# manoskary/analysisgnn

Measured on AMD Instinct MI355X. Metric: subgraph-nodes/sec fwd+bwd, HybridGNN L=3 H=256, higher is better.
Workload: dtype f32; 1 GPU; C2 (sampled, the batch a training step sees): HybridGNN L=3 H=256 out=128, 21 task heads, 32 neighbour-sampled subgraphs x (500 target notes + [5,5] hops) per GPU, per-hop counts passed (every layer trimmed); 16335 notes, 104099 edges per GPU; train step = fwd + objective (wloss) + bwd + allreduce + clip + AdamW, CSR rebuilt every step; hipGraph replay; workload_id=c2s, per_gpu_subgraphs=32, objective=wloss, parallelism=dp1, allreduce=none (one rank)

## Files before the change

### analysisgnn_amd/csrc/wgrad.hip

```cpp
#include "agnn_common.h"

namespace {

using agnn::f32x16;

struct WgArgs {
  const float* dy;
  const float* x;
  int64_t ld_dy, ld_x;
  int32_t n, out_f, in_f;
  int32_t rows_per_slice;
  int32_t tiles_in;
  float* slab;
  float* slab_b;
  int32_t out_pad, in_pad;
};

__device__ __forceinline__ void wgrad_tile(const WgArgs& a, const int tile, const int slice) {
  const int lane = threadIdx.x & 63;
  const int wave = threadIdx.x >> 6;
  const int wm = wave >> 1, wn = wave & 1;
  const int to = tile / a.tiles_in, ti = tile - to * a.tiles_in;
  const int kk = lane >> 5, c32 = lane & 31;
  const int ocol = to * 128 + wm * 64 + 2 * c32;
  const int icol = ti * 128 + wn * 64 + 2 * c32;
  const bool o_ok = ocol < a.out_f;
  const bool i_ok = icol < a.in_f;
  const int r0 = slice * a.rows_per_slice;
  int r1 = r0 + a.rows_per_slice;
  if (r1 > a.n) r1 = a.n;

  f32x16 acc00 = {0}, acc01 = {0}, acc10 = {0}, acc11 = {0};
  float bs0 = 0.f, bs1 = 0.f;
  const float* dy_s = a.dy + static_cast<int64_t>(r0) * a.ld_dy;
  const float* x_s = a.x + static_cast<int64_t>(r0) * a.ld_x;
  const uint32_t ldb_dy = static_cast<uint32_t>(a.ld_dy) * 4u, ldb_x = static_cast<uint32_t>(a.ld_x) * 4u;
  const uint32_t cb_dy = (o_ok ? ocol : 0) * 4u, cb_x = (i_ok ? icol : 0) * 4u;
  const int rel_last = a.n - 1 - r0;
  constexpr int CH = 8;
  constexpr int STEP = 2 * CH;
  float2 a0[CH], b0[CH], a1[CH], b1[CH], a2[CH], b2[CH];
  uint32_t o_dy = static_cast<uint32_t>(kk) * ldb_dy + cb_dy, o_x = static_cast<uint32_t>(kk) * ldb_x + cb_x;
  const uint32_t s_dy = 2u * ldb_dy, s_x = 2u * ldb_x;
  auto fetch_fast = [&](float2* ao, float2* bo) {
#pragma unroll
    for (int u = 0; u < CH; ++u) {
      ao[u] = *reinterpret_cast<const float2*>(reinterpret_cast<const char*>(dy_s) + o_dy);
      bo[u] = *reinterpret_cast<const float2*>(reinterpret_cast<const char*>(x_s) + o_x);
      o_dy += s_dy;
      o_x += s_x;
    }
    __builtin_amdgcn_sched_barrier(0);
  };
// ... 46 lines not shown
    fetch_fast(a1, b1);
    mma(a2, b2);
  }
  for (; c + 3 <= nfull; c += 3) {
    fetch(c + 2, a2, b2);
    mma(a0, b0);
    fetch(c + 3, a0, b0);
    mma(a1, b1);
    fetch(c + 4, a1, b1);
    mma(a2, b2);
  }
  fetch(c + 2, a2, b2);
  if (c < nchunks) mma_tail(c, a0, b0);
  if (c + 1 < nchunks) mma_tail(c + 1, a1, b1);
  if (c + 2 < nchunks) mma_tail(c + 2, a2, b2);
  float* slab = a.slab + (static_cast<int64_t>(slice) * a.out_pad) * a.in_pad;
  const int ob = to * 128 + wm * 64, ib = ti * 128 + wn * 64;
#pragma unroll
  for (int r = 0; r < 16; ++r) {
    const int i = agnn::d_row32(r, kk);
    float* row0 = slab + static_cast<int64_t>(ob + 2 * i) * a.in_pad + ib + 2 * c32;
    float* row1 = row0 + a.in_pad;
    *reinterpret_cast<float2*>(row0) = make_float2(acc00[r], acc01[r]);
    *reinterpret_cast<float2*>(row1) = make_float2(acc10[r], acc11[r]);
  }
  if (a.slab_b != nullptr && wn == 0) {
    bs0 += __shfl_xor(bs0, 32, 64);
    bs1 += __shfl_xor(bs1, 32, 64);
    if (kk == 0 && ti == 0)
      *reinterpret_cast<float2*>(a.slab_b + static_cast<int64_t>(slice) * a.out_pad + ocol) = make_float2(bs0, bs1);
  }
}

__global__ __launch_bounds__(256) void k_wgrad(WgArgs a) { wgrad_tile(a, blockIdx.x, blockIdx.y); }

constexpr int kWgBatchMax = AGNN_WGRAD_BATCH_MAX_ITEMS;

struct WgBatch {
  WgArgs it[kWgBatchMax];
  int32_t first[kWgBatchMax + 1];
  int32_t tiles[kWgBatchMax];
  int32_t n;
};

__global__ __launch_bounds__(256) void k_wgrad_batch(WgBatch b) {
  int i = 0;
  const int blk = blockIdx.x;
  while (i + 1 < b.n && blk >= b.first[i + 1]) ++i;
  const int local = blk - b.first[i];
  const int tiles = b.tiles[i];
  const int slice = local / tiles;
  wgrad_tile(b.it[i], local - slice * tiles, slice);
}


template <typename StoreW, typename StoreB>
__device__ __forceinline__ void wgrad_reduce_sums(const float* __restrict__ slab, const float* __restrict__ slab_b, int S, int out_f, int in_f,
                                                  int out_pad, int in_pad, const bool with_bias, const int block, const int n_blocks,
                                                  StoreW store_w, StoreB store_b) {
  __shared__ float2 part[8][32];
  const int col = threadIdx.x & 31, sg = threadIdx.x >> 5;
  const int half_in = in_f >> 1;
  const int64_t total = static_cast<int64_t>(out_f) * half_in;
  const int64_t plane = static_cast<int64_t>(out_pad) * in_pad;
  for (int64_t e0 = static_cast<int64_t>(block) * 32; e0 < total; e0 += static_cast<int64_t>(n_blocks) * 32) {
    const int64_t e = e0 + col;
    float2 s = make_float2(0.f, 0.f);
    int o = 0, i = 0;
    if (e < total) {
      o = static_cast<int>(e / half_in);
      i = static_cast<int>(e - static_cast<int64_t>(o) * half_in) * 2;
      const float* p = slab + static_cast<int64_t>(o) * in_pad + i;
      for (int k = sg; k < S; k += 8) {
        const float2 v = *reinterpret_cast<const float2*>(p + k * plane);
        s.x += v.x;
        s.y += v.y;
      }
    }
    part[sg][col] = s;
    __syncthreads();
    if (sg == 0 && e < total) {
      float2 t = part[0][col];
#pragma unroll
      for (int g = 1; g < 8; ++g) { t.x += part[g][col].x; t.y += part[g][col].y; }
      store_w(o, i, t);
// ... 61 lines not shown
};

Plan make_plan(int64_t n, int out_f, int in_f) {
  Plan p;
  p.tiles_out = (out_f + 127) / 128;
  p.tiles_in = (in_f + 127) / 128;
  p.out_pad = p.tiles_out * 128;
  p.in_pad = p.tiles_in * 128;
  const int tiles = p.tiles_out * p.tiles_in;
  int64_t S = 512 / tiles;
  const int64_t max_s = (n + 63) / 64;
  if (S > max_s) S = max_s;
  if (S > 64) S = 64;
  if (S < 1) S = 1;
  int64_t rps = (n + S - 1) / S;
  rps = (rps + 1) & ~int64_t{1};
  p.rows_per_slice = static_cast<int>(rps);
  p.S = static_cast<int>((n + rps - 1) / rps);
  return p;
}

}

int agnn::launch_slab_reduce(const float* slab, const float* slab_b, int S, int out_f, int in_f, int out_pad, int in_pad,
                             float* dw, int64_t ld_dw, float* db, hipStream_t s) {
  const int64_t total = static_cast<int64_t>(out_f) * (in_f >> 1);
  int blocks = static_cast<int>((total + 31) / 32);
  if (blocks > 4096) blocks = 4096;
  if (blocks < 1) blocks = 1;
  hipLaunchKernelGGL(k_wgrad_reduce, dim3(blocks), dim3(256), 0, s, slab, slab_b, S, out_f, in_f, out_pad, in_pad, dw, ld_dw, db);
  return check_launch("slab_reduce");
}

extern "C" size_t agnn_wgrad_workspace_bytes(int64_t n, int32_t out_f, int32_t in_f) {
  if (n <= 0 || out_f <= 0 || in_f <= 0) return 0;
  const Plan p = make_plan(n, out_f, in_f);
  return (static_cast<size_t>(p.S) * p.out_pad * p.in_pad + static_cast<size_t>(p.S) * p.out_pad) * sizeof(float) + 256;
}

extern "C" int agnn_wgrad_f32(const float* dy, int64_t ld_dy, const float* x, int64_t ld_x, int64_t n, int32_t out_f,
                              int32_t in_f, float* dw, int64_t ld_dw, float* db, void* workspace, size_t workspace_bytes,
                              agnn_stream_t stream_) {
  using namespace agnn;
  if (n <= 0 || n >= (int64_t{1} << 31) || out_f <= 0 || in_f <= 0) return fail(AGNN_EINVAL, "wgrad: bad sizes n=%lld out=%d in=%d", (long long)n, out_f, in_f);
  if ((out_f & 1) || (in_f & 1) || (ld_dy & 1) || (ld_x & 1) || (ld_dw & 1)) return fail(AGNN_EALIGN, "wgrad: widths and leading dimensions must be even");
  if (!dy || !x || !dw || !workspace) return fail(AGNN_EINVAL, "wgrad: null argument");
  if ((reinterpret_cast<uintptr_t>(dy) | reinterpret_cast<uintptr_t>(x) | reinterpret_cast<uintptr_t>(dw) | reinterpret_cast<uintptr_t>(db)) & 7u)
    return fail(AGNN_EALIGN, "wgrad: pointers must be 8-byte aligned");
  if (ld_dy < out_f || ld_x < in_f || ld_dw < in_f) return fail(AGNN_EINVAL, "wgrad: leading dimension smaller than the width");
  const size_t need = agnn_wgrad_workspace_bytes(n, out_f, in_f);
  if (workspace_bytes < need) return fail(AGNN_ENOMEM, "wgrad: workspace %zu < %zu bytes", workspace_bytes, need);
  const Plan p = make_plan(n, out_f, in_f);
  if ((static_cast<int64_t>(p.rows_per_slice) + 128) * (ld_dy > ld_x ? ld_dy : ld_x) * 4 >= (int64_t{1} << 32))
    return fail(AGNN_EINVAL, "wgrad: a row slice (%d rows x ld) exceeds the kernel's 32-bit byte offsets", p.rows_per_slice);
  char* ws = reinterpret_cast<char*>((reinterpret_cast<uintptr_t>(workspace) + 255) & ~uintptr_t{255});
  float* slab = reinterpret_cast<float*>(ws);
  float* slab_b = slab + static_cast<size_t>(p.S) * p.out_pad * p.in_pad;
  WgArgs a{dy, x, ld_dy, ld_x, static_cast<int32_t>(n), out_f, in_f, p.rows_per_slice, p.tiles_in, slab,
           db ? slab_b : nullptr, p.out_pad, p.in_pad};
  hipStream_t s = static_cast<hipStream_t>(stream_);
  hipLaunchKernelGGL(k_wgrad, dim3(p.tiles_out * p.tiles_in, p.S), dim3(256), 0, s, a);
  if (int rc = check_launch("wgrad")) return rc;
  return launch_slab_reduce(slab, db ? slab_b : nullptr, p.S, out_f, in_f, p.out_pad, p.in_pad, dw, ld_dw, db, s);
}

namespace {
struct BatchPlan {
  int n;
  int tiles_out[kWgBatchMax], tiles_in[kWgBatchMax], S[kWgBatchMax], rps[kWgBatchMax];
  size_t slab_off[kWgBatchMax], slabb_off[kWgBatchMax], total_floats;
};

int batch_plan(int n_items, const agnn_wgrad_item_t* items, BatchPlan& bp) {
  using namespace agnn;
  if (n_items <= 0 || n_items > kWgBatchMax || !items) return fail(AGNN_EINVAL, "wgrad_batch: %d items (1 .. %d)", n_items, kWgBatchMax);
  bp.n = n_items;
  int64_t tiles = 0;
  for (int i = 0; i < n_items; ++i) {
    const agnn_wgrad_item_t& it = items[i];
    if (it.n <= 0 || it.n >= (int64_t{1} << 31) || it.out_f <= 0 || it.in_f <= 0) return fail(AGNN_EINVAL, "wgrad_batch: item %d: bad sizes", i);
    bp.tiles_out[i] = (it.out_f + 127) / 128;
    bp.tiles_in[i] = (it.in_f + 127) / 128;
    tiles += static_cast<int64_t>(bp.tiles_out[i]) * bp.tiles_in[i];
  }
  int64_t S = 384 / tiles;
  if (S > 64) S = 64;
  if (S < 1) S = 1;
  size_t off = 0;
  for (int i = 0; i < n_items; ++i) {
    const agnn_wgrad_item_t& it = items[i];
    int64_t s_i = S;
    const int64_t max_s = (it.n + 63) / 64;
    if (s_i > max_s) s_i = max_s;
    int64_t rps = (it.n + s_i - 1) / s_i;
// ... 25 lines not shown
  if (int rc = batch_plan(n_items, items, bp)) return rc;
  if (!workspace || workspace_bytes < bp.total_floats * sizeof(float) + 256) return fail(AGNN_ENOMEM, "wgrad_batch: workspace too small");
  float* ws = reinterpret_cast<float*>((reinterpret_cast<uintptr_t>(workspace) + 255) & ~uintptr_t{255});
  WgBatch wb{};
  RedBatch rb{};
  wb.n = rb.n = n_items;
  int wg = 0, red = 0;
  for (int i = 0; i < n_items; ++i) {
    const agnn_wgrad_item_t& it = items[i];
    if ((it.out_f & 1) || (it.in_f & 1) || (it.ld_dy & 1) || (it.ld_x & 1) || (it.ld_dw & 1)) return fail(AGNN_EALIGN, "wgrad_batch: item %d: widths and leading dimensions must be even", i);
    if (!it.dy || !it.x || !it.dw) return fail(AGNN_EINVAL, "wgrad_batch: item %d: null argument", i);
    if ((reinterpret_cast<uintptr_t>(it.dy) | reinterpret_cast<uintptr_t>(it.x) | reinterpret_cast<uintptr_t>(it.dw) | reinterpret_cast<uintptr_t>(it.db)) & 7u)
      return fail(AGNN_EALIGN, "wgrad_batch: item %d: pointers must be 8-byte aligned", i);
    if (it.ld_dy < it.out_f || it.ld_x < it.in_f || it.ld_dw < it.in_f) return fail(AGNN_EINVAL, "wgrad_batch: item %d: leading dimension smaller than the width", i);
    if ((static_cast<int64_t>(bp.rps[i]) + 128) * (it.ld_dy > it.ld_x ? it.ld_dy : it.ld_x) * 4 >= (int64_t{1} << 32))
      return fail(AGNN_EINVAL, "wgrad_batch: item %d: a row slice (%d rows x ld) exceeds the kernel's 32-bit byte offsets", i, bp.rps[i]);
    const int out_pad = bp.tiles_out[i] * 128, in_pad = bp.tiles_in[i] * 128;
    float* slab = ws + bp.slab_off[i];
    float* slab_b = ws + bp.slabb_off[i];
    wb.it[i] = WgArgs{it.dy, it.x, it.ld_dy, it.ld_x, static_cast<int32_t>(it.n), it.out_f, it.in_f, bp.rps[i], bp.tiles_in[i], slab,
                      it.db ? slab_b : nullptr, out_pad, in_pad};
    wb.tiles[i] = bp.tiles_out[i] * bp.tiles_in[i];
    wb.first[i] = wg;
    wg += wb.tiles[i] * bp.S[i];
    rb.it[i] = RedItem{slab, it.db ? slab_b : nullptr, it.dw, it.db, it.ld_dw, bp.S[i], it.out_f, it.in_f, out_pad, in_pad};
    rb.first[i] = red;
    int64_t blocks = (static_cast<int64_t>(it.out_f) * (it.in_f >> 1) + 31) / 32;
    if (blocks > 1024) blocks = 1024;
    red += static_cast<int>(blocks);
  }
  wb.first[n_items] = wg;
  rb.first[n_items] = red;
  hipStream_t s = static_cast<hipStream_t>(stream_);
  hipLaunchKernelGGL(k_wgrad_batch, dim3(static_cast<unsigned>(wg)), dim3(256), 0, s, wb);
  if (int rc = check_launch("wgrad_batch")) return rc;
  hipLaunchKernelGGL(k_wgrad_reduce_batch, dim3(static_cast<unsigned>(red)), dim3(256), 0, s, rb);
  return check_launch("wgrad_batch(reduce)");
}

namespace {

constexpr int kEpiRecMax = 64;
constexpr int kEpiDbMax = 48;
constexpr int kEpiSumMax = AGNN_GRAD_MAX_SUMS;
constexpr int kEpiPartRows = 1024;

struct EpiRec {
  float* p;
  int32_t ld, c0, c1, scalar;
};
struct EpiItem {
  const float* slab;
  const float* slab_b;
  int32_t S, out_f, in_f, out_pad, in_pad;
  int16_t rec0, rec1, db0, db1;
};
struct EpiSum {
  const float* part;
  float* dgamma;
  float* dbeta;
  int32_t n_rows, H;
};
struct EpiBatch {
  EpiItem it[kWgBatchMax];
  EpiRec rec[kEpiRecMax];
  float* db[kEpiDbMax];
  EpiSum sum[kEpiSumMax];
  int32_t first[kWgBatchMax + kEpiSumMax + 1];
// ... 70 lines not shown
  int64_t ld;
  int32_t rows, cols;
  int32_t item, c0, c1;
};

bool spans_overlap(const EpiSpan& a, const EpiSpan& b) {
  const float* a_end = a.p + static_cast<int64_t>(a.rows - 1) * a.ld + a.cols;
  const float* b_end = b.p + static_cast<int64_t>(b.rows - 1) * b.ld + b.cols;
  if (a_end <= b.p || b_end <= a.p) return false;
  if (a.rows > 1 && b.rows > 1 && a.ld == b.ld) {
    int64_t r = (b.p - a.p) % a.ld;
    if (r < 0) r += a.ld;
    if (r >= a.cols && r + b.cols <= a.ld) return false;
  }
  return true;
}

}

static void epi_as_wgrad(int32_t n_items, const agnn_grad_item_t* items, agnn_wgrad_item_t* out) {
  for (int i = 0; i < n_items; ++i) {
    const agnn_grad_item_t& g = items[i];
    out[i] = agnn_wgrad_item_t{g.dy, g.x, nullptr, nullptr, g.ld_dy, g.ld_x, g.in_f, g.n, g.out_f, g.in_f};
  }
}

extern "C" size_t agnn_grad_epilogue_workspace_bytes(int32_t n_items, const agnn_grad_item_t* items) {
  if (n_items <= 0 || n_items > kWgBatchMax || !items) return 0;
  agnn_wgrad_item_t w[kWgBatchMax];
  epi_as_wgrad(n_items, items, w);
  return agnn_wgrad_batch_workspace_bytes(n_items, w);
}

extern "C" int agnn_grad_epilogue_f32(int32_t n_items, const agnn_grad_item_t* items, int32_t n_sums, const agnn_colsum_item_t* sums,
                                      void* workspace, size_t workspace_bytes, agnn_stream_t stream_) {
  using namespace agnn;
  if (n_items < 0 || n_items > kWgBatchMax || (n_items > 0 && !items)) return fail(AGNN_EINVAL, "grad_epilogue: %d products (0 .. %d)", n_items, kWgBatchMax);
  if (n_sums < 0 || n_sums > kEpiSumMax || (n_sums > 0 && !sums)) return fail(AGNN_EINVAL, "grad_epilogue: %d column sums (0 .. %d)", n_sums, kEpiSumMax);
  if (n_items == 0 && n_sums == 0) return AGNN_OK;
  BatchPlan bp;
  bp.n = 0;
  bp.total_floats = 0;
  float* ws = nullptr;
  if (n_items > 0) {
    agnn_wgrad_item_t w[kWgBatchMax];
    epi_as_wgrad(n_items, items, w);
    if (int rc = batch_plan(n_items, w, bp)) return rc;
    if (!workspace || workspace_bytes < bp.total_floats * sizeof(float) + 256) return fail(AGNN_ENOMEM, "grad_epilogue: workspace too small");
    ws = reinterpret_cast<float*>((reinterpret_cast<uintptr_t>(workspace) + 255) & ~uintptr_t{255});
  }
  static thread_local EpiSpan spans[kWgBatchMax * 2 * AGNN_PACK_MAX_SRC + 2 * kEpiSumMax];
  int n_spans = 0;
  for (int i = 0; i < n_items; ++i) {
    const agnn_grad_item_t& it = items[i];
    if ((it.out_f & 1) || (it.in_f & 1) || (it.ld_dy & 1) || (it.ld_x & 1)) return fail(AGNN_EALIGN, "grad_epilogue: item %d: widths and leading dimensions must be even", i);
    if (!it.dy || !it.x) return fail(AGNN_EINVAL, "grad_epilogue: item %d: null argument", i);
    if ((reinterpret_cast<uintptr_t>(it.dy) | reinterpret_cast<uintptr_t>(it.x)) & 7u) return fail(AGNN_EALIGN, "grad_epilogue: item %d: pointers must be 8-byte aligned", i);
    if (it.ld_dy < it.out_f || it.ld_x < it.in_f) return fail(AGNN_EINVAL, "grad_epilogue: item %d: leading dimension smaller than the width", i);
    if ((static_cast<int64_t>(bp.rps[i]) + 128) * (it.ld_dy > it.ld_x ? it.ld_dy : it.ld_x) * 4 >= (int64_t{1} << 32))
      return fail(AGNN_EINVAL, "grad_epilogue: item %d: a row slice (%d rows x ld) exceeds the kernel's 32-bit byte offsets", i, bp.rps[i]);
    if (it.n_dw < 0 || it.n_dw > AGNN_PACK_MAX_SRC || it.n_db < 0 || it.n_db > AGNN_PACK_MAX_SRC || it.n_dw + it.n_db == 0)
      return fail(AGNN_EINVAL, "grad_epilogue: item %d: %d weight and %d bias destinations (0 .. %d each, one at least)", i, it.n_dw, it.n_db, AGNN_PACK_MAX_SRC);
    for (int k = 0; k < it.n_dw; ++k) {
      const agnn_grad_dst_t& d = it.dw[k];
      const int cols = d.c1 - d.c0;
      if (!d.p || d.c0 < 0 || cols <= 0 || d.c1 > it.in_f || d.ld < cols || d.ld >= (int64_t{1} << 31))
        return fail(AGNN_EINVAL, "grad_epilogue: item %d: destination %d: columns [%d, %d) of %d, ld %lld", i, k, d.c0, d.c1, it.in_f, (long long)d.ld);
      if (reinterpret_cast<uintptr_t>(d.p) & 3u) return fail(AGNN_EALIGN, "grad_epilogue: item %d: destination %d is not a float pointer", i, k);
      if (!(cols & 1) && ((d.c0 & 1) || (d.ld & 1) || (reinterpret_cast<uintptr_t>(d.p) & 7u)))
        return fail(AGNN_EALIGN, "grad_epilogue: item %d: destination %d: an even column block needs an even c0, an even ld and an 8-byte aligned pointer", i, k);
      spans[n_spans++] = EpiSpan{d.p, d.ld, it.out_f, cols, i, d.c0, d.c1};
    }
    for (int k = 0; k < it.n_db; ++k) {
      if (!it.db[k]) return fail(AGNN_EINVAL, "grad_epilogue: item %d: null bias destination %d", i, k);
      if (reinterpret_cast<uintptr_t>(it.db[k]) & 3u) return fail(AGNN_EALIGN, "grad_epilogue: item %d: bias destination %d is not a float pointer", i, k);
      spans[n_spans++] = EpiSpan{it.db[k], it.out_f, 1, it.out_f, -1, 0, 0};
    }
  }
  for (int i = 0; i < n_sums; ++i) {
    const agnn_colsum_item_t& it = sums[i];
    if (it.n <= 0 || it.H <= 0 || (it.H & 3) || it.H > 2048 || !it.workspace || !it.dgamma || !it.dbeta)
      return fail(AGNN_EINVAL, "grad_epilogue: column sum %d: bad sizes or null argument", i);
    if (it.workspace_bytes < static_cast<size_t>(kEpiPartRows) * 2 * it.H * sizeof(float)) return fail(AGNN_ENOMEM, "grad_epilogue: column sum %d: workspace too small", i);
    if ((reinterpret_cast<uintptr_t>(it.dgamma) | reinterpret_cast<uintptr_t>(it.dbeta) | reinterpret_cast<uintptr_t>(it.workspace)) & 3u)
      return fail(AGNN_EALIGN, "grad_epilogue: column sum %d: misaligned", i);
    spans[n_spans++] = EpiSpan{it.dgamma, it.H, 1, it.H, -1, 0, 0};
    spans[n_spans++] = EpiSpan{it.dbeta, it.H, 1, it.H, -1, 0, 0};
  }
  for (int a = 0; a < n_spans; ++a)
    for (int c = a + 1; c < n_spans; ++c) {
      const EpiSpan &sa = spans[a], &sc = spans[c];
      if (sa.item >= 0 && sa.item == sc.item && sa.c0 == sc.c0 && sa.c1 == sc.c1 && sa.p == sc.p && sa.ld == sc.ld) continue;
      if (spans_overlap(sa, sc)) return fail(AGNN_EINVAL, "grad_epilogue: destinations %d and %d of the call overlap", a, c);
    }
  hipStream_t s = static_cast<hipStream_t>(stream_);
  if (n_items > 0) {
    WgBatch wb{};
    wb.n = n_items;
    int wg = 0;
    for (int i = 0; i < n_items; ++i) {
      const agnn_grad_item_t& it = items[i];
      const int out_pad = bp.tiles_out[i] * 128, in_pad = bp.tiles_in[i] * 128;
      wb.it[i] = WgArgs{it.dy, it.x, it.ld_dy, it.ld_x, static_cast<int32_t>(it.n), it.out_f, it.in_f, bp.rps[i], bp.tiles_in[i], ws + bp.slab_off[i],
                        it.n_db > 0 ? ws + bp.slabb_off[i] : nullptr, out_pad, in_pad};
      wb.tiles[i] = bp.tiles_out[i] * bp.tiles_in[i];
      wb.first[i] = wg;
      wg += wb.tiles[i] * bp.S[i];
    }
    wb.first[n_items] = wg;
    hipLaunchKernelGGL(k_wgrad_batch, dim3(static_cast<unsigned>(wg)), dim3(256), 0, s, wb);
    if (int rc = check_launch("grad_epilogue(products)")) return rc;
  }
  int at = 0;
  do {
    EpiBatch eb{};
    int n = 0, n_rec = 0, n_db = 0, blocks = 0;
    while (at < n_items && n_rec + items[at].n_dw <= kEpiRecMax && n_db + items[at].n_db <= kEpiDbMax) {
      const agnn_grad_item_t& it = items[at];
      EpiItem& e = eb.it[n];
      e.slab = ws + bp.slab_off[at];
      e.slab_b = it.n_db > 0 ? ws + bp.slabb_off[at] : nullptr;
      e.S = bp.S[at];
      e.out_f = it.out_f;
      e.in_f = it.in_f;
      e.out_pad = bp.tiles_out[at] * 128;
      e.in_pad = bp.tiles_in[at] * 128;
      e.rec0 = static_cast<int16_t>(n_rec);
      for (int k = 0; k < it.n_dw; ++k) {
        const agnn_grad_dst_t& d = it.dw[k];
        eb.rec[n_rec++] = EpiRec{d.p, static_cast<int32_t>(d.ld), d.c0, d.c1, (d.c1 - d.c0) & 1};
      }
      e.rec1 = static_cast<int16_t>(n_rec);
      e.db0 = static_cast<int16_t>(n_db);
      for (int k = 0; k < it.n_db; ++k) eb.db[n_db++] = it.db[k];
      e.db1 = static_cast<int16_t>(n_db);
      eb.first[n] = blocks;
      int64_t rb = (static_cast<int64_t>(it.out_f) * (it.in_f >> 1) + 31) / 32;
      if (rb > 1024) rb = 1024;
      blocks += static_cast<int>(rb);
      ++n;
      ++at;
    }
    eb.n_items = n;
    if (at == n_items)
      for (int i = 0; i < n_sums; ++i) {
        const agnn_colsum_item_t& it = sums[i];
        int nb = static_cast<int>((it.n + 3) / 4);
        if (nb > kEpiPartRows) nb = kEpiPartRows;
        eb.sum[i] = EpiSum{static_cast<const float*>(it.workspace), it.dgamma, it.dbeta, nb, it.H};
        eb.first[n++] = blocks;
        blocks += (2 * it.H + 31) / 32;
      }
    eb.first[n] = blocks;
    eb.n_all = n;
    if (blocks > 0) {
      hipLaunchKernelGGL(k_grad_epilogue, dim3(static_cast<unsigned>(blocks)), dim3(256), 0, s, eb);
      if (int rc = check_launch("grad_epilogue(reduce)")) return rc;
    }
  } while (at < n_items);
  return AGNN_OK;
}
```

### analysisgnn_amd/linear.py

```python
from __future__ import annotations

from typing import Optional

import torch
import torch.nn as nn
import torch.nn.functional as F

from . import _lib, resident

MIN_ROWS = 2048
MAX_OUT_IN = 512 * 1024
ENABLED = True


_WG = {"enabled": False, "scope": "all", "dirty": set()}


def enable_wgrad_overlap(flag: bool = True, scope="all") -> None:
    _WG["enabled"] = bool(flag)
    _WG["scope"] = scope if scope == "all" else frozenset([scope] if isinstance(scope, str) else scope)


def wgrad_overlap_enabled() -> bool:
    return _WG["enabled"]
# ... 281 lines not shown
    members = getattr(t, "_agnn_rowcat", None)
    return list(members) if members else None


def grad_slot_groups(groups, shapes, ok=None):
    if any(g is None for g in groups):
        return None
    from .params import adjacent
    merged = []

    def build(views):
        it = iter(views)
        for g, shape in zip(groups, shapes):
            vs = [next(it) for _ in g]
            if not vs:
                merged.append(None)
                continue
            n = 1
            for d in shape:
                n *= int(d)
            if sum(v.numel() for v in vs) != n or (len(vs) > 1 and not adjacent(vs)):
                return False
            strides, acc = [], 1
            for d in reversed(shape):
                strides.append(acc)
                acc *= int(d)
            merged.append(vs[0].as_strided(tuple(int(d) for d in shape), tuple(reversed(strides)), vs[0].storage_offset()))
        return ok is None or bool(ok(merged))
    if grad_slots([p for g in groups for p in g], build) is None:
        return None
    return merged


def _ok(t: torch.Tensor) -> bool:
    return (t.dtype == torch.float32 and t.dim() == 2 and t.stride(1) == 1 and t.stride(0) % 2 == 0
            and t.shape[1] % 2 == 0 and t.data_ptr() % 8 == 0)


def _dw_ok(dw: torch.Tensor) -> bool:
    return dw.dim() == 2 and dw.stride(1) == 1 and dw.stride(0) >= dw.shape[1] and dw.stride(0) % 2 == 0 and dw.data_ptr() % 8 == 0


def weight_grad(dy: torch.Tensor, x: torch.Tensor, want_bias: bool, dw_out: Optional[torch.Tensor] = None,
                db_out: Optional[torch.Tensor] = None):
    n, out_f = dy.shape
    in_f = x.shape[1]
    in_k = in_f
    if in_f & 1 and x.dim() == 2 and x.stride(1) == 1 and x.stride(0) > in_f:
        in_k = in_f + 1
        x = x.as_strided((n, in_k), (x.stride(0), 1), x.storage_offset())
    if not (ENABLED and dy.is_cuda and n >= MIN_ROWS and out_f * in_k <= MAX_OUT_IN and _ok(dy) and _ok(x)):
        if in_k != in_f:
            x = x[:, :in_f]
        if dw_out is not None:
            torch.mm(dy.t(), x, out=dw_out)
            if want_bias:
                torch.sum(dy, dim=0, out=db_out)
            return dw_out, (db_out if want_bias else None)
        return dy.t() @ x, (dy.sum(dim=0) if want_bias else None)
    lib = _lib.load()
    dev = dy.device
    if dw_out is not None:
        if in_k != in_f or tuple(dw_out.shape) != (out_f, in_f) or not _dw_ok(dw_out) or (want_bias and (db_out is None or not db_out.is_contiguous())):
            raise _lib.AgnnError("weight_grad: dw_out / db_out must be [out, in] (rows contiguous, even stride) / contiguous [out] with an even `in`")
        dw, db = dw_out, (db_out if want_bias else None)
    else:
        dw = torch.empty((out_f, in_k), dtype=torch.float32, device=dev)
        db = torch.empty((out_f,), dtype=torch.float32, device=dev) if want_bias else None
    nws = int(lib.agnn_wgrad_workspace_bytes(n, out_f, in_k))
    ws = torch.empty(nws, dtype=torch.uint8, device=dev)
    _lib.check(lib.agnn_wgrad_f32(dy.data_ptr(), dy.stride(0), x.data_ptr(), x.stride(0), n, out_f, in_k, dw.data_ptr(),
                                  dw.stride(0), _lib.ptr(db), ws.data_ptr(), nws, _lib.stream_ptr(dev)), "agnn_wgrad_f32")
    return (dw if in_k == in_f else dw[:, :in_f].contiguous()), db


class WgItem:
    __slots__ = ("dy", "x", "want_bias", "dw_out", "db_out", "event", "follows", "dsts", "db_dsts")

    def __init__(self, dy, x, want_bias, dw_out, db_out, follows=False, dsts=None, db_dsts=()):
        self.dy, self.x, self.want_bias, self.dw_out, self.db_out, self.event = dy, x, bool(want_bias), dw_out, db_out, None
        self.follows = bool(follows)
        self.dsts, self.db_dsts = dsts, tuple(db_dsts)

    def tensors(self):
        if self.dsts is not None:
            return (self.dy, self.x, *[d for _, _, d in self.dsts], *self.db_dsts)
        return (self.dy, self.x, self.dw_out, self.db_out)

    def destinations(self):
        if self.dsts is not None:
            return self.dsts, self.db_dsts
        return [(0, self.x.shape[1], self.dw_out)], ((self.db_out,) if self.want_bias else ())

    def __call__(self):
        if self.dsts is None:
            weight_grad(self.dy, self.x, self.want_bias, dw_out=self.dw_out, db_out=self.db_out)
            return
        from .params import pack
        dw, db = weight_grad(self.dy, self.x, self.want_bias)
        items = [(d, [dw[:, c0:c1]]) for c0, c1, d in self.dsts] + [(d.view(1, -1), [db.view(1, -1)]) for d in self.db_dsts]
        pack(items, self.dy.device)


class ColsumItem:
    __slots__ = ("ws", "n", "H", "dgamma", "dbeta", "event")

    def __init__(self, ws, n, H, dgamma, dbeta):
        self.ws, self.n, self.H, self.dgamma, self.dbeta, self.event = ws, int(n), int(H), dgamma, dbeta, None

    def tensors(self):
        return (self.ws, self.dgamma, self.dbeta)

    def __call__(self):
        _lib.check(_lib.load().agnn_norm_act_colsum_f32(self.ws.data_ptr(), self.ws.numel(), self.n, self.H, self.dgamma.data_ptr(),
                                                        self.dbeta.data_ptr(), _lib.stream_ptr(self.ws.device)), "agnn_norm_act_colsum_f32")


def colsum_batch(items) -> None:
    if not BATCH or len(items) == 1:
        for it in items:
            it()
        return
    lib = _lib.load()
    for i in range(0, len(items), _lib.WGRAD_BATCH_MAX):
        grp = items[i:i + _lib.WGRAD_BATCH_MAX]
        arr = (_lib.ColsumItem * len(grp))()
        for a, it in zip(arr, grp):
            a.workspace, a.workspace_bytes, a.n, a.H = it.ws.data_ptr(), it.ws.numel(), it.n, it.H
            a.dgamma, a.dbeta = it.dgamma.data_ptr(), it.dbeta.data_ptr()
        _lib.check(lib.agnn_norm_act_colsum_batch_f32(len(grp), arr, _lib.stream_ptr(grp[0].ws.device)), "agnn_norm_act_colsum_batch_f32")


BATCH = True


def weight_grad_batch(items) -> None:
    lib = None
    group = []
    products = 0

    def fits(it):
        n, out_f = it.dy.shape
        in_f = it.x.shape[1]
        return (BATCH and ENABLED and it.dy.is_cuda and it.dy.dim() == 2 and it.x.dim() == 2 and n >= MIN_ROWS and out_f * in_f <= MAX_OUT_IN and in_f % 2 == 0
                and _ok(it.dy) and _ok(it.x) and it.dw_out is not None and tuple(it.dw_out.shape) == (out_f, in_f) and _dw_ok(it.dw_out)
                and (not it.want_bias or (it.db_out is not None and it.db_out.is_contiguous() and it.db_out.data_ptr() % 8 == 0)))

    def run(group):
        if len(group) == 1:
            group[0]()
            return
        nonlocal lib
        lib = lib or _lib.load()
        dev = group[0].dy.device
        arr = (_lib.WgradItem * len(group))()
        for a, it in zip(arr, group):
            a.dy, a.x, a.dw = it.dy.data_ptr(), it.x.data_ptr(), it.dw_out.data_ptr()
            a.db = it.db_out.data_ptr() if it.want_bias else None
            a.ld_dy, a.ld_x, a.ld_dw, a.n = it.dy.stride(0), it.x.stride(0), it.dw_out.stride(0), it.dy.shape[0]
            a.out_f, a.in_f = it.dy.shape[1], it.x.shape[1]
        nws = int(lib.agnn_wgrad_batch_workspace_bytes(len(group), arr))
        ws = torch.empty(nws, dtype=torch.uint8, device=dev)
        _lib.check(lib.agnn_wgrad_batch_f32(len(group), arr, ws.data_ptr(), nws, _lib.stream_ptr(dev)), "agnn_wgrad_batch_f32")

    for it in items:
        if fits(it):
            joins = it.follows and group and group[-1].dy is it.dy
            if group and ((products == _lib.WGRAD_BATCH_MAX and not joins) or len(group) == _lib.WGRAD_BATCH_MAX_ITEMS):
                run(group)
                group, products, joins = [], 0, False
            group.append(it)
            products += 0 if joins else 1
        else:
            it()
    if group:
        run(group)


def _dst_ok(d: torch.Tensor, out_f: int, c0: int, c1: int) -> bool:
    cols = c1 - c0
    if d.dtype != torch.float32 or d.dim() != 2 or tuple(d.shape) != (out_f, cols) or d.stride(1) != 1 or d.stride(0) < cols:
        return False
    return d.data_ptr() % 4 == 0 if cols & 1 else (c0 % 2 == 0 and d.stride(0) % 2 == 0 and d.data_ptr() % 8 == 0)


def grad_epilogue(items, sums) -> None:
    lib = _lib.load()

    def fits(it):
        n, out_f = it.dy.shape
        in_f = it.x.shape[1]
        dsts, dbs = it.destinations()
        return (ENABLED and it.dy.is_cuda and it.dy.dim() == 2 and it.x.dim() == 2 and n >= MIN_ROWS and out_f * in_f <= MAX_OUT_IN and in_f % 2 == 0
                and _ok(it.dy) and _ok(it.x) and 0 < len(dsts) <= _lib.PACK_MAX_SRC and len(dbs) <= _lib.PACK_MAX_SRC
                and all(d is not None and _dst_ok(d, out_f, c0, c1) for c0, c1, d in dsts) and bool(dbs) == it.want_bias
                and all(d is not None and d.is_contiguous() and tuple(d.shape) == (out_f,) for d in dbs)
                and (it.dsts is not None or all(d.data_ptr() % 8 == 0 for d in dbs)))

    groups, group, products = [], [], 0
    for it in items:
        if fits(it):
            joins = it.follows and group and group[-1].dy is it.dy
            if group and ((products == _lib.WGRAD_BATCH_MAX and not joins) or len(group) == _lib.WGRAD_BATCH_MAX_ITEMS):
                groups.append(group)
                group, products, joins = [], 0, False
            group.append(it)
            products += 0 if joins else 1
        else:
            it()
    if group:
        groups.append(group)
    sums = list(sums)
    batched = [g for g in groups if len(g) > 1]
    for g in groups:
        if len(g) == 1:
            g[0]()
            continue
        take, sums = (sums[:_lib.GRAD_MAX_SUMS], sums[_lib.GRAD_MAX_SUMS:]) if g is batched[-1] else ([], sums)
        _epilogue_call(lib, g, take)
    while sums:
        _epilogue_call(lib, [], sums[:_lib.GRAD_MAX_SUMS])
        sums = sums[_lib.GRAD_MAX_SUMS:]


def _epilogue_call(lib, group, sums) -> None:
    dev = (group[0].dy if group else sums[0].ws).device
    arr = (_lib.GradItem * max(len(group), 1))()
    for a, it in zip(arr, group):
        dsts, dbs = it.destinations()
        a.dy, a.x = it.dy.data_ptr(), it.x.data_ptr()
        a.ld_dy, a.ld_x, a.n = it.dy.stride(0), it.x.stride(0), it.dy.shape[0]
        a.out_f, a.in_f = it.dy.shape[1], it.x.shape[1]
        a.n_dw, a.n_db = len(dsts), len(dbs)
        for k, (c0, c1, d) in enumerate(dsts):
            a.dw[k].p, a.dw[k].ld, a.dw[k].c0, a.dw[k].c1 = d.data_ptr(), (d.stride(0) if d.shape[0] > 1 else max(d.shape[1], d.stride(0))), c0, c1
        for k, d in enumerate(dbs):
            a.db[k] = d.data_ptr()
    sarr = (_lib.ColsumItem * max(len(sums), 1))()
    for a, it in zip(sarr, sums):
        a.workspace, a.workspace_bytes, a.n, a.H = it.ws.data_ptr(), it.ws.numel(), it.n, it.H
        a.dgamma, a.dbeta = it.dgamma.data_ptr(), it.dbeta.data_ptr()
    nws = int(lib.agnn_grad_epilogue_workspace_bytes(len(group), arr)) if group else 0
    ws = torch.empty(nws, dtype=torch.uint8, device=dev) if group else None
    _lib.check(lib.agnn_grad_epilogue_f32(len(group), arr, len(sums), sarr, _lib.ptr(ws), nws, _lib.stream_ptr(dev)), "agnn_grad_epilogue_f32")


def _leaf_slots(groups, out_f: int, in_f: int, odd_ok: bool = False):
    if groups is None or not groups[0]:
        return None

    def ok(v):
        dw, db = v
        return (_dw_ok(dw) or (odd_ok and dw.shape[1] & 1 and dw.stride(1) == 1)) and (db is None or db.data_ptr() % 8 == 0)
    v = grad_slot_groups(groups, ((out_f, in_f), (out_f,)), ok)
    return None if v is None else (v[0], v[1])


HAND_GEMM = True
HAND_GEMM_DX = False
HAND_GEMM_MIN_ROWS = 4096
HAND_GEMM_MIN_K, HAND_GEMM_MIN_N = 256, 256
HAND_GEMM_MAX_K = 1536


def _hand_gemm_dx_ok(dy, w) -> bool:
    return (dy.is_cuda and dy.dim() == 2 and dy.dtype == torch.float32 and w.dtype == torch.float32 and dy.shape[0] >= HAND_GEMM_MIN_ROWS
            and w.shape[1] % 64 == 0 and w.shape[0] % 16 == 0 and dy.stride(1) == 1 and w.stride(1) == 1 and dy.stride(0) % 4 == 0
            and w.stride(0) % 4 == 0 and dy.stride(0) >= dy.shape[1] and w.stride(0) >= w.shape[1] and dy.data_ptr() % 16 == 0 and w.data_ptr() % 16 == 0)


def _hand_gemm_ok(x, w, b) -> bool:
    return (x.is_cuda and x.dim() == 2 and x.dtype == torch.float32 and w.dtype == torch.float32 and x.shape[0] >= HAND_GEMM_MIN_ROWS
            and HAND_GEMM_MIN_K <= x.shape[1] <= HAND_GEMM_MAX_K and w.shape[0] >= HAND_GEMM_MIN_N and w.shape[0] % 64 == 0 and x.shape[1] % 16 == 0 and x.stride(1) == 1 and w.stride(1) == 1 and x.stride(0) % 4 == 0
            and w.stride(0) % 4 == 0 and x.stride(0) >= x.shape[1] and w.stride(0) >= w.shape[1] and x.data_ptr() % 16 == 0 and w.data_ptr() % 16 == 0 and (b is None or (b.dtype == torch.float32 and b.is_contiguous())))


# ... 194 lines not shown
```

### include/agnn.h

```cpp
#ifndef AGNN_H_
#define AGNN_H_

#include <stddef.h>
#include <stdint.h>

#ifdef __cplusplus
extern "C" {
#endif

typedef void* agnn_stream_t;

#define AGNN_OK        0
#define AGNN_EINVAL  (-22)
#define AGNN_EALIGN  (-14)
#define AGNN_ENOMEM  (-12)
#define AGNN_ERUNTIME (-5)

#define AGNN_MAX_SEG 32

const char* agnn_last_error(void);
int agnn_version(void);

typedef struct {
  const int64_t* row;
// ... 174 lines not shown
  int32_t H;
  float* dgamma;
  float* dbeta;
} agnn_colsum_item_t;
int agnn_norm_act_colsum_batch_f32(int32_t n_items, const agnn_colsum_item_t* items , agnn_stream_t stream);

size_t agnn_skip_act_workspace_bytes(void);
int agnn_skip_act_fwd_f32(const float* x, int64_t ld_x, const float* o, int64_t ld_o, const float* skip, int64_t n, int32_t H, float p,
                          uint32_t flags, const int64_t* rng_state, uint32_t call_id, float* z, int64_t ld_z, int64_t* rng_used,
                          agnn_stream_t stream);
int agnn_skip_act_bwd_f32(const float* x, int64_t ld_x, const float* o, int64_t ld_o, const float* skip, int64_t n, int32_t H, float p,
                          uint32_t flags, const int64_t* rng_state, uint32_t call_id, const float* dz, int64_t ld_dz, float* dx,
                          int64_t ld_dx, float* dout, int64_t ld_do, float* dskip, void* workspace, size_t workspace_bytes,
                          agnn_stream_t stream);
int agnn_norm_act_colsum_f32(const void* workspace, size_t workspace_bytes, int64_t n, int32_t H, float* dgamma, float* dbeta,
                             agnn_stream_t stream);

size_t agnn_wgrad_workspace_bytes(int64_t n, int32_t out_f, int32_t in_f);
int agnn_wgrad_f32(const float* dy, int64_t ld_dy, const float* x, int64_t ld_x, int64_t n, int32_t out_f,
                   int32_t in_f, float* dw, int64_t ld_dw, float* db, void* workspace, size_t workspace_bytes,
                   agnn_stream_t stream);
#define AGNN_WGRAD_BATCH_MAX_ITEMS 24
typedef struct {
  const float* dy;
  const float* x;
  float* dw;
  float* db;
  int64_t ld_dy, ld_x, ld_dw, n;
  int32_t out_f, in_f;
} agnn_wgrad_item_t;
size_t agnn_wgrad_batch_workspace_bytes(int32_t n_items, const agnn_wgrad_item_t* items );
int agnn_wgrad_batch_f32(int32_t n_items, const agnn_wgrad_item_t* items , void* workspace, size_t workspace_bytes,
                         agnn_stream_t stream);

#define AGNN_PACK_MAX_SRC   8
#define AGNN_PACK_MAX_ITEMS 24
typedef struct {
  float* dst;
  const float* src[AGNN_PACK_MAX_SRC];
  int64_t ld_dst, ld_src;
  int32_t rows, cols, n_src, vec_ok;
} agnn_pack_item_t;
int agnn_pack_f32(int32_t n_items, const agnn_pack_item_t* items , agnn_stream_t stream);

#define AGNN_GRAD_MAX_SUMS 16
typedef struct {
  float* p;
  int64_t ld;
  int32_t c0, c1;
} agnn_grad_dst_t;
typedef struct {
  const float* dy;
  const float* x;
  int64_t ld_dy, ld_x, n;
  int32_t out_f, in_f;
  int32_t n_dw, n_db;
  agnn_grad_dst_t dw[AGNN_PACK_MAX_SRC];
  float* db[AGNN_PACK_MAX_SRC];
} agnn_grad_item_t;
size_t agnn_grad_epilogue_workspace_bytes(int32_t n_items, const agnn_grad_item_t* items );
int agnn_grad_epilogue_f32(int32_t n_items, const agnn_grad_item_t* items , int32_t n_sums,
                           const agnn_colsum_item_t* sums , void* workspace, size_t workspace_bytes, agnn_stream_t stream);

#define AGNN_GATHER_MAX_ITEMS 128
typedef struct {
  float* dst;
  const float* src;
  int64_t n;
} agnn_gather_item_t;
int agnn_gather_f32(int32_t n_items, const agnn_gather_item_t* items , agnn_stream_t stream);

int agnn_debug_stamp(uint64_t* slot , agnn_stream_t stream);

#define AGNN_EMBED_MAX_TABLES 4
int agnn_embed_cat_fwd_f32(const float* x, int64_t ld_x, int32_t in_x, int64_t n_rows, int32_t n_tab,
                           const int64_t* const* idx , const float* const* tables ,
                           const int32_t* vocab , int32_t dim, float* out, int64_t ld_out, agnn_stream_t stream);
size_t agnn_embed_workspace_bytes(int32_t n_tab, const int32_t* vocab , int32_t dim);
int agnn_embed_cat_bwd_f32(const float* dout, int64_t ld_dout, int32_t col0, int64_t n_rows, int32_t n_tab,
                           const int64_t* const* idx , const int32_t* vocab , int32_t dim, float* dtables,
                           void* workspace, size_t workspace_bytes, agnn_stream_t stream);

int agnn_heads_fwd_f32(const float* x, int64_t ld_x, int64_t n_rows, int32_t in_f, int32_t hidden, int32_t T, const float* w1,
                       const float* b1, const float* gamma, const float* beta, float eps, const float* w2, const float* b2,
                       const int32_t* offs_dev, const int32_t* offs_host , float* z, float* y, int64_t ld_h, float* mean,
                       float* rstd, float* logits, int64_t ld_o, agnn_stream_t stream);

int agnn_gproj_fwd_f32(const float* a, int64_t ld_a, const float* w, const float* b, const int32_t* seg_off,
                       int32_t n_groups, int32_t K, int32_t n_tiles32, int64_t n_rows, float* out, int64_t ld_out,
                       agnn_stream_t stream);
size_t agnn_gproj_workspace_bytes(int64_t n_rows, int32_t sum_c, int32_t K, int32_t n_tiles32);
int agnn_gproj_bwd_f32(const float* dout, int64_t ld_dout, const float* a, int64_t ld_a, const float* w,
                       const int32_t* seg_off, int32_t n_groups, int32_t K, int32_t n_tiles32, int32_t sum_c,
                       int64_t n_rows, float* da, int64_t ld_da, float* dw, float* db, void* workspace,
                       size_t workspace_bytes, agnn_stream_t stream);
// ... 246 lines not shown
```

Baseline: 5.720 million subgraph-nodes/s.

## Add persistent-grid wgrad launch shaping and a fused single-item dst epilogue path

Turns the wgrad product kernels into grid-stride loops so an optional cap on workgroups and an optional LDS reservation (one workgroup per CU) can shape the launch. Both knobs default to off. Adds an in-place path for a lone weight-grad item that writes straight into its destination slices through the epilogue machinery, with a larger reduce grid, instead of computing dw separately and packing it afterwards. The lone path is enabled by default and removes a separate pack/copy launch, but it adds a new code path, and the asm barrier on threadIdx may perturb codegen.

```diff
diff --git a/analysisgnn_amd/csrc/wgrad.hip b/analysisgnn_amd/csrc/wgrad.hip
--- a/analysisgnn_amd/csrc/wgrad.hip
+++ b/analysisgnn_amd/csrc/wgrad.hip
@@ -1,3 +1,5 @@
+#include <atomic>
+
 #include "agnn_common.h"
 
 namespace {
@@ -17,8 +19,10 @@
 };
 
 __device__ __forceinline__ void wgrad_tile(const WgArgs& a, const int tile, const int slice) {
-  const int lane = threadIdx.x & 63;
-  const int wave = threadIdx.x >> 6;
+  int tid = threadIdx.x;
+  asm volatile("" : "+v"(tid));
+  const int lane = tid & 63;
+  const int wave = tid >> 6;
   const int wm = wave >> 1, wn = wave & 1;
   const int to = tile / a.tiles_in, ti = tile - to * a.tiles_in;
   const int kk = lane >> 5, c32 = lane & 31;
@@ -131,7 +135,12 @@
   }
 }
 
-__global__ __launch_bounds__(256) void k_wgrad(WgArgs a) { wgrad_tile(a, blockIdx.x, blockIdx.y); }
+__global__ __launch_bounds__(256) void k_wgrad(WgArgs a, int tiles, int n_work) {
+  for (int w = blockIdx.x; w < n_work; w += gridDim.x) {
+    const int slice = w / tiles;
+    wgrad_tile(a, w - slice * tiles, slice);
+  }
+}
 
 constexpr int kWgBatchMax = AGNN_WGRAD_BATCH_MAX_ITEMS;
 
@@ -143,13 +152,62 @@
 };
 
 __global__ __launch_bounds__(256) void k_wgrad_batch(WgBatch b) {
+  const int n_work = b.first[b.n];
   int i = 0;
-  const int blk = blockIdx.x;
-  while (i + 1 < b.n && blk >= b.first[i + 1]) ++i;
-  const int local = blk - b.first[i];
-  const int tiles = b.tiles[i];
-  const int slice = local / tiles;
-  wgrad_tile(b.it[i], local - slice * tiles, slice);
+  for (int w = blockIdx.x; w < n_work; w += gridDim.x) {
+    while (i + 1 < b.n && w >= b.first[i + 1]) ++i;
+    const int local = w - b.first[i];
+    const int tiles = b.tiles[i];
+    const int slice = local / tiles;
+    wgrad_tile(b.it[i], local - slice * tiles, slice);
+  }
+}
+
+constexpr unsigned kHoldLds = 84u * 1024u;
+std::atomic<int> g_cap{0}, g_one_per_cu{0};
+constexpr int kMaxDev = 64;
+std::atomic<bool> g_lds_ok[kMaxDev];
+
+unsigned capped_grid(int n_work) {
+  const int cap = g_cap.load(std::memory_order_relaxed);
+  if (cap <= 0 || n_work <= cap) return static_cast<unsigned>(n_work);
+  const int rounds = (n_work + cap - 1) / cap;
+  return static_cast<unsigned>((n_work + rounds - 1) / rounds);
+}
+
+int allow_hold_lds() {
+  using namespace agnn;
+  int dev = 0;
+  if (hipGetDevice(&dev) != hipSuccess || dev < 0 || dev >= kMaxDev) return fail(AGNN_ERUNTIME, "wgrad_launch_shape: no current HIP device");
+  if (g_lds_ok[dev].load()) return AGNN_OK;
+  hipError_t e = hipFuncSetAttribute(reinterpret_cast<const void*>(k_wgrad), hipFuncAttributeMaxDynamicSharedMemorySize, static_cast<int>(kHoldLds));
+  if (e == hipSuccess) e = hipFuncSetAttribute(reinterpret_cast<const void*>(k_wgrad_batch), hipFuncAttributeMaxDynamicSharedMemorySize, static_cast<int>(kHoldLds));
+  if (e != hipSuccess) return fail(AGNN_ERUNTIME, "wgrad_launch_shape: %u bytes of dynamic LDS refused: %s", kHoldLds, hipGetErrorString(e));
+  g_lds_ok[dev].store(true);
+  return AGNN_OK;
+}
+
+int hold_lds(hipStream_t s, unsigned* bytes) {
+  using namespace agnn;
+  *bytes = 0;
+  if (!g_one_per_cu.load(std::memory_order_relaxed)) return AGNN_OK;
+  int dev = 0;
+  if (hipGetDevice(&dev) != hipSuccess || dev < 0 || dev >= kMaxDev) return fail(AGNN_ERUNTIME, "wgrad: no current HIP device");
+  if (!g_lds_ok[dev].load()) {
+    hipStreamCaptureStatus st = hipStreamCaptureStatusNone;
+    if (hipStreamIsCapturing(s, &st) != hipSuccess || st != hipStreamCaptureStatusNone)
+      return fail(AGNN_ERUNTIME, "wgrad: one workgroup per CU was not set up on device %d before this capture (call agnn_wgrad_launch_shape there first)", dev);
+    if (int rc = allow_hold_lds()) return rc;
+  }
+  *bytes = kHoldLds;
+  return AGNN_OK;
+}
+
+int launch_products(const WgBatch& wb, hipStream_t s, const char* what) {
+  unsigned lds = 0;
+  if (int rc = hold_lds(s, &lds)) return rc;
+  hipLaunchKernelGGL(k_wgrad_batch, dim3(capped_grid(wb.first[wb.n])), dim3(256), lds, s, wb);
+  return agnn::check_launch(what);
 }
 
 
@@ -277,6 +335,16 @@
   return check_launch("slab_reduce");
 }
 
+extern "C" int agnn_wgrad_launch_shape(int32_t max_workgroups, int32_t one_per_cu) {
+  using namespace agnn;
+  if (max_workgroups < 0 || one_per_cu < 0) return fail(AGNN_EINVAL, "wgrad_launch_shape: max_workgroups=%d one_per_cu=%d (both >= 0)", max_workgroups, one_per_cu);
+  if (one_per_cu)
+    if (int rc = allow_hold_lds()) return rc;
+  g_cap.store(max_workgroups);
+  g_one_per_cu.store(one_per_cu ? 1 : 0);
+  return AGNN_OK;
+}
+
 extern "C" size_t agnn_wgrad_workspace_bytes(int64_t n, int32_t out_f, int32_t in_f) {
   if (n <= 0 || out_f <= 0 || in_f <= 0) return 0;
   const Plan p = make_plan(n, out_f, in_f);
@@ -304,7 +372,10 @@
   WgArgs a{dy, x, ld_dy, ld_x, static_cast<int32_t>(n), out_f, in_f, p.rows_per_slice, p.tiles_in, slab,
            db ? slab_b : nullptr, p.out_pad, p.in_pad};
   hipStream_t s = static_cast<hipStream_t>(stream_);
-  hipLaunchKernelGGL(k_wgrad, dim3(p.tiles_out * p.tiles_in, p.S), dim3(256), 0, s, a);
+  const int tiles = p.tiles_out * p.tiles_in, n_work = tiles * p.S;
+  unsigned lds = 0;
+  if (int rc = hold_lds(s, &lds)) return rc;
+  hipLaunchKernelGGL(k_wgrad, dim3(capped_grid(n_work)), dim3(256), lds, s, a, tiles, n_work);
   if (int rc = check_launch("wgrad")) return rc;
   return launch_slab_reduce(slab, db ? slab_b : nullptr, p.S, out_f, in_f, p.out_pad, p.in_pad, dw, ld_dw, db, s);
 }
@@ -396,8 +467,7 @@
   wb.first[n_items] = wg;
   rb.first[n_items] = red;
   hipStream_t s = static_cast<hipStream_t>(stream_);
-  hipLaunchKernelGGL(k_wgrad_batch, dim3(static_cast<unsigned>(wg)), dim3(256), 0, s, wb);
-  if (int rc = check_launch("wgrad_batch")) return rc;
+  if (int rc = launch_products(wb, s, "wgrad_batch")) return rc;
   hipLaunchKernelGGL(k_wgrad_reduce_batch, dim3(static_cast<unsigned>(red)), dim3(256), 0, s, rb);
   return check_launch("wgrad_batch(reduce)");
 }
@@ -534,8 +604,39 @@
   return agnn_wgrad_batch_workspace_bytes(n_items, w);
 }
 
+namespace {
+int single_plan(const agnn_wgrad_item_t& it, BatchPlan& bp) {
+  using namespace agnn;
+  if (it.n <= 0 || it.n >= (int64_t{1} << 31) || it.out_f <= 0 || it.in_f <= 0) return fail(AGNN_EINVAL, "wgrad_dst: bad sizes n=%lld out=%d in=%d", (long long)it.n, it.out_f, it.in_f);
+  const Plan p = make_plan(it.n, it.out_f, it.in_f);
+  bp.n = 1;
+  bp.tiles_out[0] = p.tiles_out;
+  bp.tiles_in[0] = p.tiles_in;
+  bp.S[0] = p.S;
+  bp.rps[0] = p.rows_per_slice;
+  bp.slab_off[0] = 0;
+  bp.slabb_off[0] = static_cast<size_t>(p.S) * p.out_pad * p.in_pad;
+  bp.total_floats = bp.slabb_off[0] + static_cast<size_t>(p.S) * p.out_pad;
+  return AGNN_OK;
+}
+
+int grad_epilogue(int32_t n_items, const agnn_grad_item_t* items, int32_t n_sums, const agnn_colsum_item_t* sums, void* workspace,
+                  size_t workspace_bytes, agnn_stream_t stream_, const bool single);
+}
+
 extern "C" int agnn_grad_epilogue_f32(int32_t n_items, const agnn_grad_item_t* items, int32_t n_sums, const agnn_colsum_item_t* sums,
                                       void* workspace, size_t workspace_bytes, agnn_stream_t stream_) {
+  return grad_epilogue(n_items, items, n_sums, sums, workspace, workspace_bytes, stream_, false);
+}
+
+extern "C" int agnn_wgrad_dst_f32(const agnn_grad_item_t* item, void* workspace, size_t workspace_bytes, agnn_stream_t stream_) {
+  if (!item) return agnn::fail(AGNN_EINVAL, "wgrad_dst: null argument");
+  return grad_epilogue(1, item, 0, nullptr, workspace, workspace_bytes, stream_, true);
+}
+
+namespace {
+int grad_epilogue(int32_t n_items, const agnn_grad_item_t* items, int32_t n_sums, const agnn_colsum_item_t* sums, void* workspace,
+                  size_t workspace_bytes, agnn_stream_t stream_, const bool single) {
   using namespace agnn;
   if (n_items < 0 || n_items > kWgBatchMax || (n_items > 0 && !items)) return fail(AGNN_EINVAL, "grad_epilogue: %d products (0 .. %d)", n_items, kWgBatchMax);
   if (n_sums < 0 || n_sums > kEpiSumMax || (n_sums > 0 && !sums)) return fail(AGNN_EINVAL, "grad_epilogue: %d column sums (0 .. %d)", n_sums, kEpiSumMax);
@@ -547,7 +648,7 @@
   if (n_items > 0) {
     agnn_wgrad_item_t w[kWgBatchMax];
     epi_as_wgrad(n_items, items, w);
-    if (int rc = batch_plan(n_items, w, bp)) return rc;
+    if (int rc = single ? single_plan(w[0], bp) : batch_plan(n_items, w, bp)) return rc;
     if (!workspace || workspace_bytes < bp.total_floats * sizeof(float) + 256) return fail(AGNN_ENOMEM, "grad_epilogue: workspace too small");
     ws = reinterpret_cast<float*>((reinterpret_cast<uintptr_t>(workspace) + 255) & ~uintptr_t{255});
   }
@@ -610,8 +711,7 @@
       wg += wb.tiles[i] * bp.S[i];
     }
     wb.first[n_items] = wg;
-    hipLaunchKernelGGL(k_wgrad_batch, dim3(static_cast<unsigned>(wg)), dim3(256), 0, s, wb);
-    if (int rc = check_launch("grad_epilogue(products)")) return rc;
+    if (int rc = launch_products(wb, s, "grad_epilogue(products)")) return rc;
   }
   int at = 0;
   do {
@@ -638,7 +738,8 @@
       e.db1 = static_cast<int16_t>(n_db);
       eb.first[n] = blocks;
       int64_t rb = (static_cast<int64_t>(it.out_f) * (it.in_f >> 1) + 31) / 32;
-      if (rb > 1024) rb = 1024;
+      const int64_t rb_max = single ? 4096 : 1024;
+      if (rb > rb_max) rb = rb_max;
       blocks += static_cast<int>(rb);
       ++n;
       ++at;
@@ -662,3 +763,4 @@
   } while (at < n_items);
   return AGNN_OK;
 }
+}
diff --git a/analysisgnn_amd/linear.py b/analysisgnn_amd/linear.py
--- a/analysisgnn_amd/linear.py
+++ b/analysisgnn_amd/linear.py
@@ -337,6 +337,19 @@
     return merged
 
 
+WGRAD_GRID_CAP = 0
+WGRAD_ONE_PER_CU = 0
+_SHAPE_SENT = [(0, 0)]
+
+
+def send_wgrad_launch_shape(lib=None) -> None:
+    want = (int(WGRAD_GRID_CAP), int(WGRAD_ONE_PER_CU))
+    if want != _SHAPE_SENT[0]:
+        lib = lib or _lib.load()
+        _lib.check(lib.agnn_wgrad_launch_shape(*want), "agnn_wgrad_launch_shape")
+        _SHAPE_SENT[0] = want
+
+
 def _ok(t: torch.Tensor) -> bool:
     return (t.dtype == torch.float32 and t.dim() == 2 and t.stride(1) == 1 and t.stride(0) % 2 == 0
             and t.shape[1] % 2 == 0 and t.data_ptr() % 8 == 0)
@@ -374,6 +387,7 @@
         db = torch.empty((out_f,), dtype=torch.float32, device=dev) if want_bias else None
     nws = int(lib.agnn_wgrad_workspace_bytes(n, out_f, in_k))
     ws = torch.empty(nws, dtype=torch.uint8, device=dev)
+    send_wgrad_launch_shape(lib)
     _lib.check(lib.agnn_wgrad_f32(dy.data_ptr(), dy.stride(0), x.data_ptr(), x.stride(0), n, out_f, in_k, dw.data_ptr(),
                                   dw.stride(0), _lib.ptr(db), ws.data_ptr(), nws, _lib.stream_ptr(dev)), "agnn_wgrad_f32")
     return (dw if in_k == in_f else dw[:, :in_f].contiguous()), db
@@ -400,6 +414,9 @@
     def __call__(self):
         if self.dsts is None:
             weight_grad(self.dy, self.x, self.want_bias, dw_out=self.dw_out, db_out=self.db_out)
+            return
+        if LONE_IN_PLACE and _epilogue_fits(self):
+            _epilogue_call(_lib.load(), [self], [], lone=True)
             return
         from .params import pack
         dw, db = weight_grad(self.dy, self.x, self.want_bias)
@@ -466,6 +483,7 @@
             a.out_f, a.in_f = it.dy.shape[1], it.x.shape[1]
         nws = int(lib.agnn_wgrad_batch_workspace_bytes(len(group), arr))
         ws = torch.empty(nws, dtype=torch.uint8, device=dev)
+        send_wgrad_launch_shape(lib)
         _lib.check(lib.agnn_wgrad_batch_f32(len(group), arr, ws.data_ptr(), nws, _lib.stream_ptr(dev)), "agnn_wgrad_batch_f32")
 
     for it in items:
@@ -489,19 +507,23 @@
     return d.data_ptr() % 4 == 0 if cols & 1 else (c0 % 2 == 0 and d.stride(0) % 2 == 0 and d.data_ptr() % 8 == 0)
 
 
+LONE_IN_PLACE = True
+
+
+def _epilogue_fits(it) -> bool:
+    n, out_f = it.dy.shape
+    in_f = it.x.shape[1]
+    dsts, dbs = it.destinations()
+    return (ENABLED and it.dy.is_cuda and it.dy.dim() == 2 and it.x.dim() == 2 and n >= MIN_ROWS and out_f * in_f <= MAX_OUT_IN and in_f % 2 == 0
+            and _ok(it.dy) and _ok(it.x) and 0 < len(dsts) <= _lib.PACK_MAX_SRC and len(dbs) <= _lib.PACK_MAX_SRC
+            and all(d is not None and _dst_ok(d, out_f, c0, c1) for c0, c1, d in dsts) and bool(dbs) == it.want_bias
+            and all(d is not None and d.is_contiguous() and tuple(d.shape) == (out_f,) for d in dbs)
+            and (it.dsts is not None or all(d.data_ptr() % 8 == 0 for d in dbs)))
+
+
 def grad_epilogue(items, sums) -> None:
     lib = _lib.load()
-
-    def fits(it):
-        n, out_f = it.dy.shape
-        in_f = it.x.shape[1]
-        dsts, dbs = it.destinations()
-        return (ENABLED and it.dy.is_cuda and it.dy.dim() == 2 and it.x.dim() == 2 and n >= MIN_ROWS and out_f * in_f <= MAX_OUT_IN and in_f % 2 == 0
-                and _ok(it.dy) and _ok(it.x) and 0 < len(dsts) <= _lib.PACK_MAX_SRC and len(dbs) <= _lib.PACK_MAX_SRC
-                and all(d is not None and _dst_ok(d, out_f, c0, c1) for c0, c1, d in dsts) and bool(dbs) == it.want_bias
-                and all(d is not None and d.is_contiguous() and tuple(d.shape) == (out_f,) for d in dbs)
-                and (it.dsts is not None or all(d.data_ptr() % 8 == 0 for d in dbs)))
-
+    fits = _epilogue_fits
     groups, group, products = [], [], 0
     for it in items:
         if fits(it):
@@ -528,7 +550,7 @@
         sums = sums[_lib.GRAD_MAX_SUMS:]
 
 
-def _epilogue_call(lib, group, sums) -> None:
+def _epilogue_call(lib, group, sums, lone: bool = False) -> None:
     dev = (group[0].dy if group else sums[0].ws).device
     arr = (_lib.GradItem * max(len(group), 1))()
     for a, it in zip(arr, group):
@@ -545,8 +567,16 @@
     for a, it in zip(sarr, sums):
         a.workspace, a.workspace_bytes, a.n, a.H = it.ws.data_ptr(), it.ws.numel(), it.n, it.H
         a.dgamma, a.dbeta = it.dgamma.data_ptr(), it.dbeta.data_ptr()
+    if lone:
+        it = group[0]
+        nws = int(lib.agnn_wgrad_workspace_bytes(it.dy.shape[0], it.dy.shape[1], it.x.shape[1]))
+        ws = torch.empty(nws, dtype=torch.uint8, device=dev)
+        send_wgrad_launch_shape(lib)
+        _lib.check(lib.agnn_wgrad_dst_f32(arr, ws.data_ptr(), nws, _lib.stream_ptr(dev)), "agnn_wgrad_dst_f32")
+        return
     nws = int(lib.agnn_grad_epilogue_workspace_bytes(len(group), arr)) if group else 0
     ws = torch.empty(nws, dtype=torch.uint8, device=dev) if group else None
+    send_wgrad_launch_shape(lib)
     _lib.check(lib.agnn_grad_epilogue_f32(len(group), arr, len(sums), sarr, _lib.ptr(ws), nws, _lib.stream_ptr(dev)), "agnn_grad_epilogue_f32")
 
 
diff --git a/include/agnn.h b/include/agnn.h
--- a/include/agnn.h
+++ b/include/agnn.h
@@ -230,6 +230,7 @@
 size_t agnn_wgrad_batch_workspace_bytes(int32_t n_items, const agnn_wgrad_item_t* items );
 int agnn_wgrad_batch_f32(int32_t n_items, const agnn_wgrad_item_t* items , void* workspace, size_t workspace_bytes,
                          agnn_stream_t stream);
+int agnn_wgrad_launch_shape(int32_t max_workgroups, int32_t one_per_cu);
 
 #define AGNN_PACK_MAX_SRC   8
 #define AGNN_PACK_MAX_ITEMS 24
@@ -259,6 +260,7 @@
 size_t agnn_grad_epilogue_workspace_bytes(int32_t n_items, const agnn_grad_item_t* items );
 int agnn_grad_epilogue_f32(int32_t n_items, const agnn_grad_item_t* items , int32_t n_sums,
                            const agnn_colsum_item_t* sums , void* workspace, size_t workspace_bytes, agnn_stream_t stream);
+int agnn_wgrad_dst_f32(const agnn_grad_item_t* item , void* workspace, size_t workspace_bytes, agnn_stream_t stream);
 
 #define AGNN_GATHER_MAX_ITEMS 128
 typedef struct {
```

Result: no change. 5.715 million subgraph-nodes/s, median of 2 (-0.1%).
